# traveller59/spconv

Measured on NVIDIA H100. Metric: active-voxels/sec fwd+bwd SubMConv3d 3^3 C=64, higher is better.
Workload: dtype fp16

## Files before the change

spconv_b200/csrc/rulebook.cu:

```cuda
#include "common.cuh"
#include "gemm.cuh"
#include "hash.cuh"
#include "rank.cuh"
#include <cub/cub.cuh>

namespace spx {
size_t radix_argsort_workspace_bytes(int64_t n);
int radix_argsort_pair(uint32_t *mask0, int32_t *argsort0, int64_t n0, uint32_t *mask1, int32_t *argsort1, int64_t n1,
                       int key_bits, void *ws0, size_t ws0_bytes, void *ws1, size_t ws1_bytes, cudaStream_t stream);
}

namespace spx {

struct Geom {
    int ndim, batch, kv;
    int in_dims[SPX_MAX_NDIM], out_dims[SPX_MAX_NDIM], ksize[SPX_MAX_NDIM];
    int stride[SPX_MAX_NDIM], padding[SPX_MAX_NDIM], dilation[SPX_MAX_NDIM];
    int transposed;
};

static Geom make_geom(const spx_conv_geometry *g, bool subm) {
    Geom r;
    memset(&r, 0, sizeof(r));
    r.ndim = g->ndim;
    r.batch = g->batch_size;
    r.kv = 1;
    r.transposed = g->transposed;
    for (int a = 0; a < g->ndim; ++a) {
        r.in_dims[a] = g->in_dims[a];
        r.ksize[a] = g->ksize[a];
        r.dilation[a] = g->dilation[a];
        r.kv *= g->ksize[a];
        if (subm) {
            r.out_dims[a] = g->in_dims[a];
            r.stride[a] = 1;
            r.padding[a] = (g->ksize[a] / 2) * g->dilation[a];
        } else {
            r.out_dims[a] = g->out_dims[a];
            r.stride[a] = g->stride[a];
            r.padding[a] = g->padding[a];
        }
    }
    return r;
}

static bool needs_i64(const Geom &g, const int *dims) {
    double v = (double)g.batch;
    for (int a = 0; a < g.ndim; ++a) v *= (double)dims[a];
    return v >= 2147483647.0;
}

__device__ __forceinline__ void load_coord(const int32_t *indices, int64_t i, int ndim, int (&c)[SPX_MAX_NDIM + 1]) {
    if (ndim == 3) {
        int4 v = __ldg(reinterpret_cast<const int4 *>(indices) + i);
        c[0] = v.x; c[1] = v.y; c[2] = v.z; c[3] = v.w;
    } else {
        const int32_t *p = indices + i * (ndim + 1);
#pragma unroll
        for (int a = 0; a <= SPX_MAX_NDIM; ++a) if (a <= ndim) c[a] = __ldg(p + a);
    }
}

__device__ __forceinline__ int64_t linear_key(const int (&c)[SPX_MAX_NDIM + 1], const int *dims, int ndim) {
    int64_t k = c[0];
#pragma unroll
    for (int a = 0; a < SPX_MAX_NDIM; ++a) if (a < ndim) k = k * dims[a] + c[a + 1];
    return k;
}

__device__ __forceinline__ void offset_taps(int k, const int *ksize, int ndim, int (&r)[SPX_MAX_NDIM]) {
#pragma unroll
    for (int a = SPX_MAX_NDIM - 1; a >= 0; --a) if (a < ndim) { r[a] = k % ksize[a]; k /= ksize[a]; }
}

template <typename Table>
__global__ void subm_insert_kernel(Table table, Geom g, const int32_t *__restrict__ indices, int64_t N) {
    int64_t i = blockIdx.x * (int64_t)blockDim.x + threadIdx.x;
    if (i >= N) return;
    int c[SPX_MAX_NDIM + 1];
    load_coord(indices, i, g.ndim, c);
    table.insert_min(linear_key(c, g.in_dims, g.ndim), (int32_t)i);
}

template <typename Table>
__global__ void subm_probe_kernel(Table table, Geom g, const int32_t *__restrict__ indices, int64_t N,
                                  int32_t *__restrict__ pair_fwd, int32_t *__restrict__ pair_bwd,
                                  uint32_t *__restrict__ mask, int words) {
    int64_t o = blockIdx.x * (int64_t)blockDim.x + threadIdx.x;
    if (o >= N) return;
    int c[SPX_MAX_NDIM + 1];
    load_coord(indices, o, g.ndim, c);
    const int kv = g.kv;
    uint32_t mword = 0;
    int r[SPX_MAX_NDIM] = {0, 0, 0, 0};
    for (int k = 0; k < kv; ++k) {
        int32_t found = -1;
        if (k == kv / 2) {
            found = (int32_t)o;
        } else {
            int q[SPX_MAX_NDIM + 1];
            q[0] = c[0];
            bool valid = c[0] >= 0 && c[0] < g.batch;
#pragma unroll
            for (int a = 0; a < SPX_MAX_NDIM; ++a) {
                if (a < g.ndim) {
                    q[a + 1] = c[a + 1] - g.padding[a] + r[a] * g.dilation[a];
                    valid = valid && q[a + 1] >= 0 && q[a + 1] < g.in_dims[a];
                }
            }
            if (valid) {
                int32_t v;
                if (table.find_slot(linear_key(q, g.in_dims, g.ndim), v) >= 0) found = v;
            }
        }
        pair_fwd[(int64_t)k * N + o] = found;
        if (pair_bwd) pair_bwd[(int64_t)(kv - 1 - k) * N + o] = found;
        if (found >= 0) mword |= 1u << (k & 31);
        if (mask && ((k & 31) == 31 || k == kv - 1)) {
            mask[o * words + (k >> 5)] = mword;
            mword = 0;
        }
#pragma unroll
        for (int a = SPX_MAX_NDIM - 1; a >= 0; --a) {
            if (a < g.ndim) {
                if (++r[a] < g.ksize[a]) break;
                r[a] = 0;
            }
        }
    }
}

constexpr int K3_VOX = 128;
constexpr int K3_PER_LANE = K3_VOX / 32;
__global__ void __launch_bounds__(27 * 32, 2)
subm_probe_k3_kernel(Table32 table, Geom g, const int32_t *__restrict__ indices, int64_t N,
                     int32_t *__restrict__ pair_fwd, int32_t *__restrict__ pair_bwd,
                     uint32_t *__restrict__ mask, int32_t *__restrict__ row_table) {
    __shared__ uint32_t hit_col[27][K3_PER_LANE];
    __shared__ int32_t row_stage[K3_VOX][27];
    const int lane = threadIdx.x & 31;
    const int k = threadIdx.x >> 5;
    const int rz = k / 9, ry = (k / 3) % 3, rx = k % 3;
    const int64_t vbase = blockIdx.x * (int64_t)K3_VOX;
    const int D0 = g.in_dims[0], D1 = g.in_dims[1], D2 = g.in_dims[2];
    const int oz = (rz - 1) * g.dilation[0], oy = (ry - 1) * g.dilation[1], ox = (rx - 1) * g.dilation[2];
    int4 c[K3_PER_LANE];
#pragma unroll
    for (int j = 0; j < K3_PER_LANE; ++j) {
        const int64_t o = vbase + j * 32 + lane;
        c[j] = o < N ? __ldg(reinterpret_cast<const int4 *>(indices) + o) : make_int4(-1, 0, 0, 0);
    }
    uint32_t key[K3_PER_LANE], h[K3_PER_LANE];
    unsigned long long cur[K3_PER_LANE];
    uint32_t pending = 0;
#pragma unroll
    for (int j = 0; j < K3_PER_LANE; ++j) {
        const int qz = c[j].y + oz, qy = c[j].z + oy, qx = c[j].w + ox;
        const bool valid = k != 13 && c[j].x >= 0 && c[j].x < g.batch && qz >= 0 && qz < D0 && qy >= 0 && qy < D1 &&
                           qx >= 0 && qx < D2;
        key[j] = (uint32_t)(((c[j].x * D0 + qz) * D1 + qy) * D2 + qx);
        h[j] = mix32(key[j]) & table.cap_mask;
        cur[j] = valid ? __ldg(&table.slots[h[j]]) : Table32::EMPTY;
    }
#pragma unroll
    for (int j = 0; j < K3_PER_LANE; ++j)
        if (cur[j] != Table32::EMPTY && (uint32_t)(cur[j] >> 32) != key[j]) pending |= 1u << j;
    while (pending) {
#pragma unroll
        for (int j = 0; j < K3_PER_LANE; ++j)
            if (pending & (1u << j)) { h[j] = (h[j] + 1) & table.cap_mask; cur[j] = __ldg(&table.slots[h[j]]); }
#pragma unroll
        for (int j = 0; j < K3_PER_LANE; ++j)
            if ((pending & (1u << j)) && (cur[j] == Table32::EMPTY || (uint32_t)(cur[j] >> 32) == key[j]))
                pending &= ~(1u << j);
    }
#pragma unroll
    for (int j = 0; j < K3_PER_LANE; ++j) {
        const int64_t o = vbase + j * 32 + lane;
        int32_t found = cur[j] != Table32::EMPTY ? (int32_t)(uint32_t)cur[j] : -1;
        if (k == 13 && o < N) found = (int32_t)o;
        if (o < N) {
            pair_fwd[(int64_t)k * N + o] = found;
            if (pair_bwd) pair_bwd[(int64_t)(26 - k) * N + o] = found;
        }
        const uint32_t hits = __ballot_sync(0xffffffffu, found >= 0);
        if (lane == 0) hit_col[k][j] = hits;
        row_stage[j * 32 + lane][k] = found;
    }
    __syncthreads();
    if (mask && threadIdx.x < K3_VOX && vbase + threadIdx.x < N) {
        const int v = threadIdx.x;
        uint32_t m = 0;
#pragma unroll
        for (int kk = 0; kk < 27; ++kk) m |= ((hit_col[kk][v >> 5] >> (v & 31)) & 1u) << kk;
        mask[vbase + v] = m;
    }
    if (row_table) {
        for (int e = threadIdx.x; e < K3_VOX * 32; e += 27 * 32) {
            const int v = e >> 5, kk = e & 31;
            if (vbase + v < N) row_table[(vbase + v) * 32 + kk] = kk < 27 ? row_stage[v][kk] : -1;
        }
    }
}

__device__ __forceinline__ bool conv_out_coord(const Geom &g, const int (&c)[SPX_MAX_NDIM + 1],
                                               const int (&r)[SPX_MAX_NDIM], int (&o)[SPX_MAX_NDIM + 1]) {
    bool valid = c[0] >= 0 && c[0] < g.batch;
    o[0] = c[0];
#pragma unroll
    for (int a = 0; a < SPX_MAX_NDIM; ++a) {
        if (a < g.ndim) {
            if (g.transposed) {
                o[a + 1] = c[a + 1] * g.stride[a] - g.padding[a] + r[a] * g.dilation[a];
                valid = valid && o[a + 1] >= 0 && o[a + 1] < g.out_dims[a];
            } else {
                int h = c[a + 1] + g.padding[a] - r[a] * g.dilation[a];
                o[a + 1] = h / g.stride[a];
                valid = valid && o[a + 1] >= 0 && o[a + 1] < g.out_dims[a] && (h % g.stride[a] == 0);
            }
        }
    }
    return valid;
}

struct Taps3 { int r0, r1, r2; };
__device__ __forceinline__ Taps3 block_taps3(const Geom &g, int k) {
    Taps3 t;
    t.r2 = k % g.ksize[2]; k /= g.ksize[2];
    t.r1 = k % g.ksize[1]; k /= g.ksize[1];
    t.r0 = k;
    return t;
}
__device__ __forceinline__ bool axis_out(int c, int pad, int r, int dil, int stride, int odim, int &o) {
    const int h = c + pad - r * dil;
// ... 390 lines not shown
    int32_t *blk = table + t * (int64_t)(kv + 1) * 128;
    const int32_t *col = pair + (src >= 0 ? src : 0);
    uint32_t rm0 = ~0u, rm1 = ~0u, rm2 = ~0u, rm3 = ~0u;
    if (mask && j < rows) {
        const uint32_t *mr = mask + j * words;
        rm0 = __ldg(mr);
        if (words > 1) rm1 = __ldg(mr + 1);
        if (words > 2) rm2 = __ldg(mr + 2);
        if (words > 3) rm3 = __ldg(mr + 3);
    }
#pragma unroll 8
    for (int k = q; k < kv; k += TT_SPLIT) {
        const uint32_t w = k < 32 ? rm0 : k < 64 ? rm1 : k < 96 ? rm2 : rm3;
        blk[k * 128 + r] = src >= 0 && ((w >> (k & 31)) & 1u) ? __ldg(col + (int64_t)k * pair_stride) : -1;
    }
    if (q == 0) blk[kv * 128 + r] = src;
    __shared__ uint32_t red[4][4];
    if (q == 0) {
        for (int w = 0; w < words; ++w) {
            uint32_t m = 0;
            if (j < rows) {
                if (mask) m = __ldg(mask + j * words + w);
                else { int hi = kv - 32 * w; m = hi >= 32 ? 0xffffffffu : ((1u << hi) - 1u); }
            }
            m = __reduce_or_sync(0xffffffffu, m);
            if ((r & 31) == 0) red[w][r >> 5] = m;
        }
    }
    __syncthreads();
    if (threadIdx.x < words) tile_mask[t * words + threadIdx.x] = red[threadIdx.x][0] | red[threadIdx.x][1] |
                                                                  red[threadIdx.x][2] | red[threadIdx.x][3];
}

__global__ void __launch_bounds__(128 * TT_SPLIT)
build_tile_table_rows_kernel(const int32_t *__restrict__ row_table, int kv, const int32_t *__restrict__ argsort,
                             const uint32_t *__restrict__ mask, int64_t rows, int32_t *__restrict__ table,
                             uint32_t *__restrict__ tile_mask) {
    const int64_t t = blockIdx.x;
    const int r = threadIdx.x & 127;
    const int q = threadIdx.x >> 7;
    const int64_t j = t * 128 + r;
    int32_t src = -1;
    if (j < rows) src = argsort ? __ldg(argsort + j) : (int32_t)j;
    int32_t *blk = table + t * (int64_t)(kv + 1) * 128;
    int4 v0 = make_int4(-1, -1, -1, -1), v1 = v0;
    if (src >= 0) {
        const int4 *rp = reinterpret_cast<const int4 *>(row_table + (int64_t)src * 32 + q * 8);
        v0 = __ldg(rp); v1 = __ldg(rp + 1);
    }
    const int32_t vals[8] = {v0.x, v0.y, v0.z, v0.w, v1.x, v1.y, v1.z, v1.w};
#pragma unroll
    for (int i = 0; i < 8; ++i) {
        const int k = q * 8 + i;
        if (k < kv) blk[k * 128 + r] = vals[i];
    }
    if (q == 0) blk[kv * 128 + r] = src;
    __shared__ uint32_t red[4];
    if (q == 0) {
        uint32_t m = 0;
        if (j < rows) m = mask ? __ldg(mask + j) : (kv >= 32 ? 0xffffffffu : ((1u << kv) - 1u));
        m = __reduce_or_sync(0xffffffffu, m);
        if ((r & 31) == 0) red[r >> 5] = m;
    }
    __syncthreads();
    if (threadIdx.x == 0) tile_mask[t] = red[0] | red[1] | red[2] | red[3];
}

constexpr int TO_THREADS = 1024;
constexpr int TO_BUCKETS = 130;
struct ToJob { const uint32_t *tile_mask; int tiles; int32_t *rec; int32_t *state; };
struct ToJobs { ToJob j[2]; };
__global__ void __launch_bounds__(TO_THREADS)
tile_order_kernel(const ToJobs jobs, int words) {
    const ToJob &J = jobs.j[blockIdx.x];
    const uint32_t *__restrict__ tile_mask = J.tile_mask;
    const int tiles = J.tiles;
    int32_t *__restrict__ rec = J.rec;
    int32_t *__restrict__ state = J.state;
    __shared__ int bucket_base[TO_BUCKETS];
    __shared__ int wcnt[TO_THREADS / 32][TO_BUCKETS];
    const int tid = threadIdx.x, lane = tid & 31, warp = tid >> 5;
    if (tid < TT_STATE_INTS) state[tid] = 0;
    for (int i = tid; i < TO_BUCKETS; i += TO_THREADS) bucket_base[i] = 0;
    __syncthreads();
    auto load_mask = [&](int t, uint32_t (&m)[4]) {
        uint32_t any = 0;
#pragma unroll
        for (int w = 0; w < 4; ++w) { m[w] = w < words ? __ldg(tile_mask + (int64_t)t * words + w) : 0u; any |= m[w]; }
        if (!any) m[0] = 1u;
        return __popc(m[0]) + __popc(m[1]) + __popc(m[2]) + __popc(m[3]);
    };
    for (int t = tid; t < tiles; t += TO_THREADS) {
        uint32_t m[4];
        atomicAdd(&bucket_base[load_mask(t, m)], 1);
    }
    __syncthreads();
    if (warp == 0) {
        int carry = 0;
        for (int base = TO_BUCKETS - 1; base >= 0; base -= 32) {
            const int c = base - lane;
            const int n = c >= 0 ? bucket_base[c] : 0;
            int incl = n;
#pragma unroll
            for (int o = 1; o < 32; o <<= 1) {
                const int up = __shfl_up_sync(0xffffffffu, incl, o);
                if (lane >= o) incl += up;
            }
            if (c >= 0) bucket_base[c] = carry + incl - n;
            carry += __shfl_sync(0xffffffffu, incl, 31);
        }
    }
    __syncthreads();
    for (int t0 = 0; t0 < tiles; t0 += TO_THREADS) {
        for (int i = tid; i < (TO_THREADS / 32) * TO_BUCKETS; i += TO_THREADS) (&wcnt[0][0])[i] = 0;
        __syncthreads();
        const int t = t0 + tid;
        const bool ok = t < tiles;
        uint32_t m[4] = {0, 0, 0, 0};
        const int c = ok ? load_mask(t, m) : TO_BUCKETS - 1;
        const unsigned peers = __match_any_sync(0xffffffffu, ok ? c : -1);
        const int rank = __popc(peers & ((1u << lane) - 1u));
        if (ok && rank == 0) wcnt[warp][c] = __popc(peers);
        __syncthreads();
        const int live_warps = min(TO_THREADS / 32, (tiles - t0 + 31) / 32);
        for (int b = tid; b < TO_BUCKETS; b += TO_THREADS) {
            int run = bucket_base[b];
            for (int w = 0; w < live_warps; ++w) { const int n = wcnt[w][b]; wcnt[w][b] = run; run += n; }
            bucket_base[b] = run;
        }
        __syncthreads();
        if (ok) {
            int32_t *r = rec + (int64_t)(wcnt[warp][c] + rank) * TT_REC_INTS;
            *reinterpret_cast<int4 *>(r) = make_int4(t, (int)m[0], (int)m[1], (int)m[2]);
            *reinterpret_cast<int4 *>(r + 4) = make_int4((int)m[3], 0, 0, 0);
        }
        __syncthreads();
    }
}

}

using namespace spx;

static int validate_geom(const spx_conv_geometry *g) {
    SPX_REQUIRE(g != nullptr, "geometry is NULL");
    SPX_REQUIRE(g->ndim >= 1 && g->ndim <= SPX_MAX_NDIM, "ndim must be in [1, %d], got %d", SPX_MAX_NDIM, g->ndim);
    SPX_REQUIRE(g->batch_size > 0, "batch_size must be positive");
    for (int a = 0; a < g->ndim; ++a) {
        SPX_REQUIRE(g->ksize[a] > 0 && g->dilation[a] > 0 && g->in_dims[a] > 0, "bad ksize/dilation/dims on axis %d", a);
    }
    return 0;
}

struct RbLayout {
    size_t table_bytes, table_vals_bytes;
    uint32_t capacity;
    bool i64;
};

static RbLayout rb_layout(const Geom &g, int64_t items, const int *dims, int factor = 4) {
    RbLayout L;
    L.i64 = needs_i64(g, dims);
    L.capacity = table_capacity(items, factor);
    L.table_bytes = (size_t)L.capacity * 8;
    L.table_vals_bytes = L.i64 ? (size_t)L.capacity * 4 : 0;
    return L;
}

extern "C" int64_t spx_conv_max_out(const spx_conv_geometry *g, int64_t num_in) {
    int64_t res = num_in, kv = 1;
    for (int i = 0; i < g->ndim; ++i) {
        kv *= g->ksize[i];
        if (g->ksize[i] > g->stride[i]) res *= (g->ksize[i] + g->stride[i] - 1) / g->stride[i];
    }
    if (g->transposed) res = kv * num_in;
    if (res > kv * num_in) res = kv * num_in;
    return res;
}

static size_t sort_pairs_temp_bytes(int64_t n) {
    cudaGetLastError();
    size_t bytes = 0;
    cudaError_t e = cub::DeviceRadixSort::SortPairs(nullptr, bytes, (const uint32_t *)nullptr, (uint32_t *)nullptr,
                                                    (const uint32_t *)nullptr, (uint32_t *)nullptr, (int)n);
    const size_t floor_bytes = (size_t)(n > 0 ? n : 1) * 16 + (1u << 20);
    if (e != cudaSuccess) { cudaGetLastError(); return floor_bytes; }
    return bytes > floor_bytes ? bytes : floor_bytes;
}

static bool subm_k3_path(const Geom &gg) {
    return !needs_i64(gg, gg.in_dims) && gg.ndim == 3 && gg.ksize[0] == 3 && gg.ksize[1] == 3 && gg.ksize[2] == 3;
}

static int subm_rulebook(const spx_conv_geometry *g, const int32_t *indices, int64_t N, int32_t *pair_fwd,
                         int32_t *pair_bwd, uint32_t *mask, int32_t *row_table, void *workspace,
                         size_t workspace_bytes, spx_stream_t stream_) {
    if (validate_geom(g)) return 2;
    for (int a = 0; a < g->ndim; ++a)
        SPX_REQUIRE(g->ksize[a] % 2 == 1, "subm only support odd ksize");
    SPX_REQUIRE(N >= 0 && N < 2147483647ll, "bad N");
    if (N == 0) return 0;
    SPX_REQUIRE(indices && pair_fwd && workspace, "NULL pointer argument");
    cudaStream_t stream = (cudaStream_t)stream_;
    Geom gg = make_geom(g, true);
    SPX_REQUIRE((int64_t)gg.kv * N < 2147483647ll * 4, "kv*N too large");
    RbLayout L = rb_layout(gg, N, gg.in_dims);
    WorkspaceCarver ws(workspace, workspace_bytes);
    void *tbl = ws.take<char>(L.table_bytes);
    int32_t *tvals = L.i64 ? ws.take<int32_t>(L.capacity) : nullptr;
    SPX_REQUIRE(ws.ok(), "rulebook workspace too small: need %zu, have %zu", ws.off, workspace_bytes);
    int words = (gg.kv + 31) / 32;
    const int T = 128;
    unsigned nblk = (unsigned)div_up64(N, T);
    SPX_CHECK_CUDA(cudaMemsetAsync(tbl, 0xFF, L.table_bytes, stream));
    if (!L.i64) {
        Table32 t{(unsigned long long *)tbl, L.capacity - 1};
        subm_insert_kernel<<<nblk, T, 0, stream>>>(t, gg, indices, N);
        SPX_CHECK_LAUNCH("subm_insert_kernel");
        if (subm_k3_path(gg)) {
            subm_probe_k3_kernel<<<(unsigned)div_up64(N, K3_VOX), 27 * 32, 0, stream>>>(t, gg, indices, N, pair_fwd,
                                                                                        pair_bwd, mask, row_table);
        } else {
            subm_probe_kernel<<<nblk, T, 0, stream>>>(t, gg, indices, N, pair_fwd, pair_bwd, mask, words);
        }
        SPX_CHECK_LAUNCH("subm_probe_kernel");
    } else {
        SPX_CHECK_CUDA(cudaMemsetAsync(tvals, 0x7F, (size_t)L.capacity * 4, stream));
        Table64 t{(long long *)tbl, tvals, L.capacity - 1};
        subm_insert_kernel<<<nblk, T, 0, stream>>>(t, gg, indices, N);
        SPX_CHECK_LAUNCH("subm_insert_kernel");
        subm_probe_kernel<<<nblk, T, 0, stream>>>(t, gg, indices, N, pair_fwd, pair_bwd, mask, words);
        SPX_CHECK_LAUNCH("subm_probe_kernel");
    }
    return 0;
}

extern "C" int spx_subm_rulebook(const spx_conv_geometry *g, const int32_t *indices, int64_t N, int32_t *pair_fwd,
                                 int32_t *pair_bwd, uint32_t *mask, void *workspace, size_t workspace_bytes,
                                 spx_stream_t stream) {
    return subm_rulebook(g, indices, N, pair_fwd, pair_bwd, mask, nullptr, workspace, workspace_bytes, stream);
}


namespace {
struct ConvWs {
    void *tbl; int32_t *tvals;
    uint32_t *slot;
    uint32_t *rank_bitmap; int *rank_tiles;
    size_t rank_bytes; int64_t rank_ntiles;
    int *counter;
    size_t bytes;
    RbLayout L;
};

struct ConvStage1Record { const void *ws; uint32_t capacity; };
thread_local ConvStage1Record g_stage1 = {nullptr, 0};

uint32_t optimistic_capacity(int64_t max_out, uint32_t full_capacity) {
    uint32_t cap = table_capacity((max_out + 3) / 4, 2);
    return cap < full_capacity ? cap : full_capacity;
}
int carve_conv_ws(const spx_conv_geometry *g, const Geom &gg, int64_t N, void *workspace, size_t bytes, ConvWs &w) {
// ... 223 lines not shown
    WorkspaceCarver ws(workspace, workspace_bytes);
    uint32_t *keys_in = ws.take<uint32_t>(N);
    uint32_t *keys_out = ws.take<uint32_t>(N);
    int32_t *perm_a = ws.take<int32_t>(N);
    int32_t *perm_b = ws.take<int32_t>(N);
    uint32_t *rows_tmp = ws.take<uint32_t>((size_t)N * words);
    size_t tmp_bytes = sort_pairs_temp_bytes(N);
    void *tmp = ws.take<char>(tmp_bytes);
    SPX_REQUIRE(ws.ok(), "argsort workspace too small: need %zu, have %zu", ws.off, workspace_bytes);
    iota_kernel<<<nblk, 256, 0, stream>>>(perm_a, N);
    SPX_CHECK_LAUNCH("iota_kernel");
    int32_t *cur = perm_a, *nxt = perm_b;
    for (int w = words - 1; w >= 0; --w) {
        gather_word_kernel<<<nblk, 256, 0, stream>>>(mask, cur, N, words, w, keys_in);
        SPX_CHECK_LAUNCH("gather_word_kernel");
        SPX_CHECK_CUDA(cub::DeviceRadixSort::SortPairs(tmp, tmp_bytes, (const uint32_t *)keys_in, keys_out,
                                                       (const int32_t *)cur, nxt, (int)N, 0, 32, stream));
        count_launch(3);
        int32_t *t = cur; cur = nxt; nxt = t;
    }
    SPX_CHECK_CUDA(cudaMemcpyAsync(argsort, cur, (size_t)N * 4, cudaMemcpyDeviceToDevice, stream));
    gather_rows_kernel<<<nblk, 256, 0, stream>>>(mask, argsort, N, words, rows_tmp);
    SPX_CHECK_LAUNCH("gather_rows_kernel");
    SPX_CHECK_CUDA(cudaMemcpyAsync(mask, rows_tmp, (size_t)N * words * 4, cudaMemcpyDeviceToDevice, stream));
    return 0;
}

extern "C" size_t spx_tile_table_elems(int64_t rows, int kv) {
    return (size_t)tt_total_elems(div_up64(rows > 0 ? rows : 1, 128), kv);
}

static int build_tile_table(const int32_t *pair, int64_t pair_stride, int kv, const int32_t *argsort,
                            const uint32_t *mask, int64_t rows, const int32_t *row_table, int32_t *table,
                            uint32_t *tile_mask, spx_stream_t stream_) {
    SPX_REQUIRE(kv >= 1 && kv <= 128, "build_tile_table: kernel volume %d not in [1,128]", kv);
    if (rows == 0) return 0;
    SPX_REQUIRE((pair || row_table) && table && tile_mask, "build_tile_table: NULL pointer argument");
    cudaStream_t stream = (cudaStream_t)stream_;
    int words = (kv + 31) / 32;
    if (row_table) {
        SPX_REQUIRE(kv <= 32, "build_tile_table: row_table holds at most 32 offsets per row, kv = %d", kv);
        SPX_REQUIRE(((uintptr_t)row_table & 15u) == 0, "build_tile_table: row_table must be 16-byte aligned");
        build_tile_table_rows_kernel<<<(unsigned)div_up64(rows, 128), 128 * TT_SPLIT, 0, stream>>>(
            row_table, kv, argsort, mask, rows, table, tile_mask);
        SPX_CHECK_LAUNCH("build_tile_table_rows_kernel");
    } else {
        TtJobs jobs;
        memset(&jobs, 0, sizeof(jobs));
        jobs.j[0] = TtJob{pair, pair_stride, argsort, mask, rows, table, tile_mask};
        build_tile_table_kernel<<<dim3((unsigned)div_up64(rows, 128), 1), 128 * TT_SPLIT, 0, stream>>>(jobs, kv, words);
        SPX_CHECK_LAUNCH("build_tile_table_kernel");
    }
    const int64_t tiles = div_up64(rows, 128);
    SPX_REQUIRE(tiles < 2147483647ll, "build_tile_table: too many tiles");
    SPX_REQUIRE(((uintptr_t)table & 15u) == 0, "build_tile_table: table must be 16-byte aligned");
    int32_t *rec = table + tt_blocks_elems(tiles, kv);
    ToJobs oj;
    memset(&oj, 0, sizeof(oj));
    oj.j[0] = ToJob{tile_mask, (int)tiles, rec, rec + tiles * TT_REC_INTS};
    tile_order_kernel<<<1, TO_THREADS, 0, stream>>>(oj, words);
    SPX_CHECK_LAUNCH("tile_order_kernel");
    return 0;
}

extern "C" int spx_build_tile_table(const int32_t *pair, int64_t pair_stride, int kv, const int32_t *argsort,
                                    const uint32_t *mask, int64_t rows, int32_t *table, uint32_t *tile_mask,
                                    spx_stream_t stream) {
    return build_tile_table(pair, pair_stride, kv, argsort, mask, rows, nullptr, table, tile_mask, stream);
}

static int build_tile_tables_pair(int kv, const int32_t *pair0, const int32_t *argsort0, const uint32_t *mask0, int64_t rows0,
                                  int32_t *table0, uint32_t *tmask0, const int32_t *pair1, const int32_t *argsort1,
                                  const uint32_t *mask1, int64_t rows1, int32_t *table1, uint32_t *tmask1,
                                  cudaStream_t stream) {
    SPX_REQUIRE(kv >= 1 && kv <= 128, "build_tile_table: kernel volume %d not in [1,128]", kv);
    const int words = (kv + 31) / 32;
    const int64_t tiles0 = div_up64(rows0, 128), tiles1 = div_up64(rows1, 128);
    SPX_REQUIRE(tiles0 < 2147483647ll && tiles1 < 2147483647ll, "build_tile_table: too many tiles");
    SPX_REQUIRE((((uintptr_t)table0 | (uintptr_t)table1) & 15u) == 0, "build_tile_table: table must be 16-byte aligned");
    TtJobs jobs;
    memset(&jobs, 0, sizeof(jobs));
    jobs.j[0] = TtJob{pair0, rows0, argsort0, mask0, rows0, table0, tmask0};
    jobs.j[1] = TtJob{pair1, rows1, argsort1, mask1, rows1, table1, tmask1};
    const int64_t tmax = tiles0 > tiles1 ? tiles0 : tiles1;
    build_tile_table_kernel<<<dim3((unsigned)tmax, 2), 128 * TT_SPLIT, 0, stream>>>(jobs, kv, words);
    SPX_CHECK_LAUNCH("build_tile_table_kernel");
    int32_t *rec0 = table0 + tt_blocks_elems(tiles0, kv), *rec1 = table1 + tt_blocks_elems(tiles1, kv);
    ToJobs oj;
    memset(&oj, 0, sizeof(oj));
    oj.j[0] = ToJob{tmask0, (int)tiles0, rec0, rec0 + tiles0 * TT_REC_INTS};
    oj.j[1] = ToJob{tmask1, (int)tiles1, rec1, rec1 + tiles1 * TT_REC_INTS};
    tile_order_kernel<<<2, TO_THREADS, 0, stream>>>(oj, words);
    SPX_CHECK_LAUNCH("tile_order_kernel");
    return 0;
}


static size_t subm_row_table_bytes(const spx_conv_geometry *g, int64_t N) {
    return subm_k3_path(make_geom(g, true)) ? align_up((size_t)N * 32 * sizeof(int32_t), 256) : 0;
}

extern "C" size_t spx_subm_rulebook_all_workspace_size(const spx_conv_geometry *g, int64_t N) {
    if (!g || g->ndim < 1 || g->ndim > SPX_MAX_NDIM) return 0;
    int kv = 1;
    for (int a = 0; a < g->ndim; ++a) kv *= g->ksize[a];
    const size_t a = spx_rulebook_workspace_size(g, N, 0, 1);
    const size_t b = spx_mask_argsort_workspace_size(N, (kv + 31) / 32);
    return align_up(a > b ? a : b, 256) + subm_row_table_bytes(g, N) + 256;
}

extern "C" int spx_subm_rulebook_all(const spx_conv_geometry *g, const int32_t *indices, int64_t N, int32_t *pair_fwd,
                                     int32_t *pair_bwd, uint32_t *mask, int32_t *argsort, int do_sort,
                                     int32_t *tile_table, uint32_t *tile_mask, void *workspace, size_t workspace_bytes,
                                     spx_stream_t stream) {
    if (validate_geom(g)) return 2;
    if (N == 0) return 0;
    SPX_REQUIRE(mask && argsort && tile_table && tile_mask && workspace, "subm_rulebook_all: NULL pointer argument");
    SPX_REQUIRE(workspace_bytes >= spx_subm_rulebook_all_workspace_size(g, N), "subm_rulebook_all: workspace too small");
    int kv = 1;
    for (int a = 0; a < g->ndim; ++a) kv *= g->ksize[a];
    const int words = (kv + 31) / 32;
    const size_t rb = spx_rulebook_workspace_size(g, N, 0, 1), as = spx_mask_argsort_workspace_size(N, words);
    const size_t shared = align_up(rb > as ? rb : as, 256);
    int32_t *row_table = subm_row_table_bytes(g, N) ? (int32_t *)((char *)workspace + shared) : nullptr;
    if (int rc = subm_rulebook(g, indices, N, pair_fwd, pair_bwd, mask, row_table, workspace, rb, stream)) return rc;
    if (int rc = spx_mask_argsort(mask, argsort, N, words, kv, do_sort, workspace, as, stream)) return rc;
    return build_tile_table(pair_fwd, N, kv, argsort, mask, N, row_table, tile_table, tile_mask, stream);
}

extern "C" size_t spx_conv_rulebook_all_workspace_size(const spx_conv_geometry *g, int64_t N) {
    if (!g || g->ndim < 1 || g->ndim > SPX_MAX_NDIM) return 0;
    int kv = 1;
    for (int a = 0; a < g->ndim; ++a) kv *= g->ksize[a];
    const int64_t max_rows = spx_conv_max_out(g, N) > N ? spx_conv_max_out(g, N) : N;
    return align_up(spx_rulebook_workspace_size(g, N, 0, 0), 256) +
           2 * align_up(spx_mask_argsort_workspace_size(max_rows, (kv + 31) / 32), 256) + 256;
}

extern "C" int spx_conv_rulebook_stage2_all(const spx_conv_geometry *g, const int32_t *indices, int64_t N, int64_t M,
                                            int32_t *out_inds, int32_t *pair_fwd, int32_t *pair_bwd, uint32_t *mask_fwd,
                                            uint32_t *mask_bwd, int32_t *argsort_fwd, int32_t *argsort_bwd, int do_sort,
                                            int32_t *table_fwd, uint32_t *tmask_fwd, int32_t *table_bwd,
                                            uint32_t *tmask_bwd, void *workspace, size_t workspace_bytes,
                                            spx_stream_t stream) {
    if (validate_geom(g)) return 2;
    if (N == 0 || M == 0) return 0;
    SPX_REQUIRE(mask_fwd && mask_bwd && argsort_fwd && table_fwd && tmask_fwd && workspace,
                "conv_rulebook_stage2_all: NULL pointer argument");
    const bool train = argsort_bwd != nullptr;
    SPX_REQUIRE((table_bwd != nullptr) == train && (tmask_bwd != nullptr) == train,
                "conv_rulebook_stage2_all: argsort_bwd, table_bwd and tmask_bwd must all be given (training) or all be "
                "NULL (inference)");
    SPX_REQUIRE(workspace_bytes >= spx_conv_rulebook_all_workspace_size(g, N), "conv_rulebook_stage2_all: workspace too small");
    int kv = 1;
    for (int a = 0; a < g->ndim; ++a) kv *= g->ksize[a];
    const int words = (kv + 31) / 32;
    const size_t rb = spx_rulebook_workspace_size(g, N, 0, 0);
    void *sort_ws = (char *)workspace + align_up(rb, 256);
    const size_t sort_bytes = workspace_bytes - align_up(rb, 256);
    if (int rc = spx_conv_rulebook_stage2(g, indices, N, M, out_inds, pair_fwd, pair_bwd, mask_fwd, mask_bwd, workspace, rb, stream)) return rc;
// ... 15 lines not shown
```

spconv_b200/csrc/sort.cu:

```cuda
#include "common.cuh"

namespace spx {

constexpr int RS_BITS = 9;
constexpr int RS_BINS = 1 << RS_BITS;
constexpr int RS_THREADS = 256;
constexpr int RS_WARPS = RS_THREADS / 32;
constexpr int RS_ITEMS = 4;
constexpr int RS_TILE = RS_THREADS * RS_ITEMS;
constexpr int RS_AGG_BITS = 11;
constexpr int RS_AGG_SLOTS = 1 << RS_AGG_BITS;
constexpr int RS_TILE_SHIFT = 10;
static_assert((1 << RS_TILE_SHIFT) == RS_TILE, "tile shift");

struct RsJob {
    const uint32_t *kin; const int32_t *vin;
    int64_t n; int nblk;
    int *counts; int *totals;
    uint32_t *kout; int32_t *vout;
    int *counts_next;
};
struct RsJobs { RsJob j[2]; };

__global__ void __launch_bounds__(RS_THREADS)
rs_hist_kernel(const RsJobs jobs, int shift) {
    const RsJob &J = jobs.j[blockIdx.y];
    if ((int)blockIdx.x >= J.nblk) return;
    const uint32_t *__restrict__ keys = J.kin;
    const int64_t n = J.n;
    const int nblk = J.nblk;
    int *__restrict__ counts = J.counts;
    __shared__ int hist[RS_BINS];
    for (int i = threadIdx.x; i < RS_BINS; i += RS_THREADS) hist[i] = 0;
    __syncthreads();
    const int64_t base = (int64_t)blockIdx.x * RS_TILE;
#pragma unroll
    for (int j = 0; j < RS_ITEMS; ++j) {
        const int64_t i = base + j * RS_THREADS + threadIdx.x;
        if (i < n) atomicAdd(&hist[(keys[i] >> shift) & (RS_BINS - 1)], 1);
    }
    __syncthreads();
    for (int d = threadIdx.x; d < RS_BINS; d += RS_THREADS) counts[(int64_t)d * nblk + blockIdx.x] = hist[d];
}

__global__ void __launch_bounds__(RS_THREADS)
rs_scan_kernel(const RsJobs jobs) {
// ... 130 lines not shown
    if (counts_next) {
        __syncthreads();
        for (int s2 = tid; s2 < RS_AGG_SLOTS; s2 += RS_THREADS)
            if (agg_cell[s2] >= 0) atomicAdd(counts_next + agg_cell[s2], agg_cnt[s2]);
    }
}

size_t radix_argsort_workspace_bytes(int64_t n) {
    const int64_t nblk = div_up64(n > 0 ? n : 1, RS_TILE);
    return 4 * align_up((size_t)n * 4, 256) + 2 * align_up((size_t)RS_BINS * nblk * 4, 256) +
           align_up(RS_BINS * 4, 256) + 1024;
}

namespace {
struct RsPlan {
    uint32_t *keys_a, *keys_b; int32_t *vals_a, *vals_b;
    int *counts_ab[2]; int *totals;
    int nblk;
};
int rs_carve(int64_t n, void *workspace, size_t bytes, RsPlan &p) {
    WorkspaceCarver ws(workspace, bytes);
    p.keys_a = ws.take<uint32_t>(n); p.vals_a = ws.take<int32_t>(n);
    p.keys_b = ws.take<uint32_t>(n); p.vals_b = ws.take<int32_t>(n);
    p.nblk = (int)div_up64(n, RS_TILE);
    p.counts_ab[0] = ws.take<int>((size_t)RS_BINS * p.nblk);
    p.counts_ab[1] = ws.take<int>((size_t)RS_BINS * p.nblk);
    p.totals = ws.take<int>(RS_BINS);
    SPX_REQUIRE(ws.ok(), "argsort workspace too small: need %zu, have %zu", ws.off, bytes);
    return 0;
}
}

int radix_argsort_pair(uint32_t *mask0, int32_t *argsort0, int64_t n0, uint32_t *mask1, int32_t *argsort1, int64_t n1,
                       int key_bits, void *ws0, size_t ws0_bytes, void *ws1, size_t ws1_bytes, cudaStream_t stream) {
    if (n0 == 0 && n1 == 0) return 0;
    if (n0 == 0) return radix_argsort_pair(mask1, argsort1, n1, nullptr, nullptr, 0, key_bits, ws1, ws1_bytes, nullptr, 0, stream);
    if (key_bits < 1) key_bits = 1;
    if (key_bits > 32) key_bits = 32;
    const int passes = (key_bits + RS_BITS - 1) / RS_BITS;
    const int njobs = n1 > 0 ? 2 : 1;
    RsPlan pl[2];
    uint32_t *masks[2] = {mask0, mask1};
    int32_t *argsorts[2] = {argsort0, argsort1};
    const int64_t ns[2] = {n0, n1};
    if (int rc = rs_carve(n0, ws0, ws0_bytes, pl[0])) return rc;
    if (njobs == 2) if (int rc = rs_carve(n1, ws1, ws1_bytes, pl[1])) return rc;
    RsJobs jobs;
    memset(&jobs, 0, sizeof(jobs));
    int max_nblk = 0;
    for (int q = 0; q < njobs; ++q) {
        jobs.j[q].kin = masks[q]; jobs.j[q].vin = nullptr; jobs.j[q].n = ns[q]; jobs.j[q].nblk = pl[q].nblk;
        jobs.j[q].totals = pl[q].totals;
        if (pl[q].nblk > max_nblk) max_nblk = pl[q].nblk;
    }
    const dim3 grid_tiles(max_nblk, njobs), grid_scan(RS_BINS, njobs);
    for (int q = 0; q < njobs; ++q) jobs.j[q].counts = pl[q].counts_ab[0];
    rs_hist_kernel<<<grid_tiles, RS_THREADS, 0, stream>>>(jobs, 0);
    SPX_CHECK_LAUNCH("rs_hist_kernel");
    for (int pass = 0; pass < passes; ++pass) {
        const bool last = pass == passes - 1;
        for (int q = 0; q < njobs; ++q) {
            RsJob &J = jobs.j[q];
            J.kout = (pass & 1) ? pl[q].keys_b : pl[q].keys_a;
            J.vout = (pass & 1) ? pl[q].vals_b : pl[q].vals_a;
            if (last && pass > 0) { J.kout = masks[q]; J.vout = argsorts[q]; }
            J.counts = pl[q].counts_ab[pass & 1];
            J.counts_next = last ? nullptr : pl[q].counts_ab[(pass + 1) & 1];
        }
        rs_scan_kernel<<<grid_scan, RS_THREADS, 0, stream>>>(jobs);
        SPX_CHECK_LAUNCH("rs_scan_kernel");
        if (pass == 0) rs_scatter_kernel<true><<<grid_tiles, RS_THREADS, 0, stream>>>(jobs, pass * RS_BITS);
        else rs_scatter_kernel<false><<<grid_tiles, RS_THREADS, 0, stream>>>(jobs, pass * RS_BITS);
        SPX_CHECK_LAUNCH("rs_scatter_kernel");
        for (int q = 0; q < njobs; ++q) { jobs.j[q].kin = jobs.j[q].kout; jobs.j[q].vin = jobs.j[q].vout; }
    }
    if (passes == 1) {
        for (int q = 0; q < njobs; ++q) {
            SPX_CHECK_CUDA(cudaMemcpyAsync(masks[q], pl[q].keys_a, (size_t)ns[q] * 4, cudaMemcpyDeviceToDevice, stream));
            SPX_CHECK_CUDA(cudaMemcpyAsync(argsorts[q], pl[q].vals_a, (size_t)ns[q] * 4, cudaMemcpyDeviceToDevice, stream));
        }
    }
    return 0;
}

}
```

spconv_b200/csrc/sparse_add.cu:

```cuda
#include "common.cuh"

namespace spx {
size_t radix_argsort_workspace_bytes(int64_t n);
int radix_argsort_pair(uint32_t *mask0, int32_t *argsort0, int64_t n0, uint32_t *mask1, int32_t *argsort1, int64_t n1,
                       int key_bits, void *ws0, size_t ws0_bytes, void *ws1, size_t ws1_bytes, cudaStream_t stream);

constexpr int SA_THREADS = 256;
constexpr int SA_MAX = SPX_SPARSE_ADD_MAX_OPERANDS;

struct SaOperands {
    int count;
    const void *features[SA_MAX];
    void *grads[SA_MAX];
    int64_t start[SA_MAX + 1];
};

__device__ __forceinline__ int operand_of(const SaOperands &ops, int64_t g) {
    int lo = 0, hi = ops.count - 1;
    while (lo < hi) {
        const int mid = (lo + hi + 1) >> 1;
        if (ops.start[mid] <= g) lo = mid;
        else hi = mid - 1;
    }
    return lo;
}

__global__ void sa_keys_kernel(const int32_t *__restrict__ dst, int64_t n, uint32_t m, uint32_t *__restrict__ keys) {
    const int64_t i = blockIdx.x * (int64_t)blockDim.x + threadIdx.x;
    if (i >= n) return;
    const int32_t o = __ldg(dst + i);
    keys[i] = o < 0 ? m : (uint32_t)o;
}

__global__ void sa_offsets_kernel(const uint32_t *__restrict__ keys, int64_t n, uint32_t m, int32_t *__restrict__ offsets) {
    const int64_t p = blockIdx.x * (int64_t)blockDim.x + threadIdx.x;
    if (p >= n) return;
    const int64_t k = keys[p];
    const int64_t prev = p == 0 ? -1 : (int64_t)keys[p - 1];
// ... 209 lines not shown
```

Before: 516.3 million.

## Fuse radix-sort histogram into subm probe and tile ordering into table build

The 3x3x3 submanifold probe kernel now builds the first-pass radix histogram of the mask in shared memory and adds it into the sort's count buffer, so the sort skips its own histogram kernel. The insert kernel zeroes that count buffer, which removes a separate memset. The tile-order step is folded into the last block of the row-table tile-build kernel using a ticket counter, removing another launch. Together these cut kernel launches and an extra pass over the mask, at the cost of extra global atomics in the probe and a single-block serial tail in the build kernel.

```diff
diff --git a/spconv_b200/csrc/rulebook.cu b/spconv_b200/csrc/rulebook.cu
--- a/spconv_b200/csrc/rulebook.cu
+++ b/spconv_b200/csrc/rulebook.cu
@@ -2,13 +2,8 @@
 #include "gemm.cuh"
 #include "hash.cuh"
 #include "rank.cuh"
+#include "sort.cuh"
 #include <cub/cub.cuh>
-
-namespace spx {
-size_t radix_argsort_workspace_bytes(int64_t n);
-int radix_argsort_pair(uint32_t *mask0, int32_t *argsort0, int64_t n0, uint32_t *mask1, int32_t *argsort1, int64_t n1,
-                       int key_bits, void *ws0, size_t ws0_bytes, void *ws1, size_t ws1_bytes, cudaStream_t stream);
-}
 
 namespace spx {
 
@@ -74,8 +69,10 @@
 }
 
 template <typename Table>
-__global__ void subm_insert_kernel(Table table, Geom g, const int32_t *__restrict__ indices, int64_t N) {
+__global__ void subm_insert_kernel(Table table, Geom g, const int32_t *__restrict__ indices, int64_t N,
+                                   int *__restrict__ zero, int64_t n_zero) {
     int64_t i = blockIdx.x * (int64_t)blockDim.x + threadIdx.x;
+    for (int64_t j = i; j < n_zero; j += (int64_t)gridDim.x * blockDim.x) zero[j] = 0;
     if (i >= N) return;
     int c[SPX_MAX_NDIM + 1];
     load_coord(indices, i, g.ndim, c);
@@ -135,9 +132,12 @@
 __global__ void __launch_bounds__(27 * 32, 2)
 subm_probe_k3_kernel(Table32 table, Geom g, const int32_t *__restrict__ indices, int64_t N,
                      int32_t *__restrict__ pair_fwd, int32_t *__restrict__ pair_bwd,
-                     uint32_t *__restrict__ mask, int32_t *__restrict__ row_table) {
+                     uint32_t *__restrict__ mask, int32_t *__restrict__ row_table, int *__restrict__ sort_counts) {
     __shared__ uint32_t hit_col[27][K3_PER_LANE];
     __shared__ int32_t row_stage[K3_VOX][27];
+    __shared__ int hist[RS_BINS];
+    if (sort_counts)
+        for (int d = threadIdx.x; d < RS_BINS; d += 27 * 32) hist[d] = 0;
     const int lane = threadIdx.x & 31;
     const int k = threadIdx.x >> 5;
     const int rz = k / 9, ry = (k / 3) % 3, rx = k % 3;
@@ -194,12 +194,19 @@
 #pragma unroll
         for (int kk = 0; kk < 27; ++kk) m |= ((hit_col[kk][v >> 5] >> (v & 31)) & 1u) << kk;
         mask[vbase + v] = m;
+        if (sort_counts) atomicAdd(&hist[m & (RS_BINS - 1)], 1);
     }
     if (row_table) {
         for (int e = threadIdx.x; e < K3_VOX * 32; e += 27 * 32) {
             const int v = e >> 5, kk = e & 31;
             if (vbase + v < N) row_table[(vbase + v) * 32 + kk] = kk < 27 ? row_stage[v][kk] : -1;
         }
+    }
+    if (sort_counts) {
+        const int sort_nblk = (int)((N + RS_TILE - 1) >> RS_TILE_SHIFT);
+        __syncthreads();
+        for (int d = threadIdx.x; d < RS_BINS; d += 27 * 32)
+            if (hist[d]) atomicAdd(sort_counts + (int64_t)d * sort_nblk + (vbase >> RS_TILE_SHIFT), hist[d]);
     }
 }
 
@@ -656,10 +663,102 @@
                                                                   red[threadIdx.x][2] | red[threadIdx.x][3];
 }
 
+constexpr int TO_THREADS = 1024;
+constexpr int TO_BUCKETS = 130;
+struct ToJob { const uint32_t *tile_mask; int tiles; int32_t *rec; int32_t *state; };
+struct ToJobs { ToJob j[2]; };
+
+template <int THREADS>
+__device__ __forceinline__ void tile_order_block(const ToJob &J, int words) {
+    static_assert(THREADS >= TT_STATE_INTS, "one thread per scheduler scratch int");
+    const uint32_t *__restrict__ tile_mask = J.tile_mask;
+    const int tiles = J.tiles;
+    int32_t *__restrict__ rec = J.rec;
+    int32_t *__restrict__ state = J.state;
+    __shared__ int bucket_base[TO_BUCKETS];
+    __shared__ int wcnt[THREADS / 32][TO_BUCKETS];
+    const int tid = threadIdx.x, lane = tid & 31, warp = tid >> 5;
+    if (tid < TT_STATE_INTS) state[tid] = 0;
+    for (int i = tid; i < TO_BUCKETS; i += THREADS) bucket_base[i] = 0;
+    __syncthreads();
+    auto load_mask = [&](int t, uint32_t (&m)[4]) {
+        uint32_t any = 0;
+#pragma unroll
+        for (int w = 0; w < 4; ++w) { m[w] = w < words ? __ldcg(tile_mask + (int64_t)t * words + w) : 0u; any |= m[w]; }
+        if (!any) m[0] = 1u;
+        return __popc(m[0]) + __popc(m[1]) + __popc(m[2]) + __popc(m[3]);
+    };
+    for (int t = tid; t < tiles; t += THREADS) {
+        uint32_t m[4];
+        atomicAdd(&bucket_base[load_mask(t, m)], 1);
+    }
+    __syncthreads();
+    if (warp == 0) {
+        int carry = 0;
+        for (int base = TO_BUCKETS - 1; base >= 0; base -= 32) {
+            const int c = base - lane;
+            const int n = c >= 0 ? bucket_base[c] : 0;
+            int incl = n;
+#pragma unroll
+            for (int o = 1; o < 32; o <<= 1) {
+                const int up = __shfl_up_sync(0xffffffffu, incl, o);
+                if (lane >= o) incl += up;
+            }
+            if (c >= 0) bucket_base[c] = carry + incl - n;
+            carry += __shfl_sync(0xffffffffu, incl, 31);
+        }
+    }
+    __syncthreads();
+    for (int t0 = 0; t0 < tiles; t0 += THREADS) {
+        for (int i = tid; i < (THREADS / 32) * TO_BUCKETS; i += THREADS) (&wcnt[0][0])[i] = 0;
+        __syncthreads();
+        const int t = t0 + tid;
+        const bool ok = t < tiles;
+        uint32_t m[4] = {0, 0, 0, 0};
+        const int c = ok ? load_mask(t, m) : TO_BUCKETS - 1;
+        const unsigned peers = __match_any_sync(0xffffffffu, ok ? c : -1);
+        const int rank = __popc(peers & ((1u << lane) - 1u));
+        if (ok && rank == 0) wcnt[warp][c] = __popc(peers);
+        __syncthreads();
+        const int live_warps = min(THREADS / 32, (tiles - t0 + 31) / 32);
+        for (int b = tid; b < TO_BUCKETS; b += THREADS) {
+            int run = bucket_base[b];
+            for (int w = 0; w < live_warps; ++w) { const int n = wcnt[w][b]; wcnt[w][b] = run; run += n; }
+            bucket_base[b] = run;
+        }
+        __syncthreads();
+        if (ok) {
+            int32_t *r = rec + (int64_t)(wcnt[warp][c] + rank) * TT_REC_INTS;
+            *reinterpret_cast<int4 *>(r) = make_int4(t, (int)m[0], (int)m[1], (int)m[2]);
+            *reinterpret_cast<int4 *>(r + 4) = make_int4((int)m[3], 0, 0, 0);
+        }
+        __syncthreads();
+    }
+}
+
+
+__global__ void __launch_bounds__(TO_THREADS)
+tile_order_kernel(const ToJobs jobs, int words) {
+    tile_order_block<TO_THREADS>(jobs.j[blockIdx.x], words);
+}
+
+__device__ __forceinline__ bool last_block_ticket(int *ticket) {
+    __shared__ int last_s;
+    __threadfence();
+    __syncthreads();
+    if (threadIdx.x == 0) {
+        last_s = atomicAdd(ticket, 1) == (int)gridDim.x - 1;
+        if (last_s) *ticket = 0;
+    }
+    __syncthreads();
+    if (last_s) __threadfence();
+    return last_s;
+}
+
 __global__ void __launch_bounds__(128 * TT_SPLIT)
 build_tile_table_rows_kernel(const int32_t *__restrict__ row_table, int kv, const int32_t *__restrict__ argsort,
                              const uint32_t *__restrict__ mask, int64_t rows, int32_t *__restrict__ table,
-                             uint32_t *__restrict__ tile_mask) {
+                             uint32_t *__restrict__ tile_mask, int *__restrict__ ticket, const ToJob order) {
     const int64_t t = blockIdx.x;
     const int r = threadIdx.x & 127;
     const int q = threadIdx.x >> 7;
@@ -688,78 +787,7 @@
     }
     __syncthreads();
     if (threadIdx.x == 0) tile_mask[t] = red[0] | red[1] | red[2] | red[3];
-}
-
-constexpr int TO_THREADS = 1024;
-constexpr int TO_BUCKETS = 130;
-struct ToJob { const uint32_t *tile_mask; int tiles; int32_t *rec; int32_t *state; };
-struct ToJobs { ToJob j[2]; };
-__global__ void __launch_bounds__(TO_THREADS)
-tile_order_kernel(const ToJobs jobs, int words) {
-    const ToJob &J = jobs.j[blockIdx.x];
-    const uint32_t *__restrict__ tile_mask = J.tile_mask;
-    const int tiles = J.tiles;
-    int32_t *__restrict__ rec = J.rec;
-    int32_t *__restrict__ state = J.state;
-    __shared__ int bucket_base[TO_BUCKETS];
-    __shared__ int wcnt[TO_THREADS / 32][TO_BUCKETS];
-    const int tid = threadIdx.x, lane = tid & 31, warp = tid >> 5;
-    if (tid < TT_STATE_INTS) state[tid] = 0;
-    for (int i = tid; i < TO_BUCKETS; i += TO_THREADS) bucket_base[i] = 0;
-    __syncthreads();
-    auto load_mask = [&](int t, uint32_t (&m)[4]) {
-        uint32_t any = 0;
-#pragma unroll
-        for (int w = 0; w < 4; ++w) { m[w] = w < words ? __ldg(tile_mask + (int64_t)t * words + w) : 0u; any |= m[w]; }
-        if (!any) m[0] = 1u;
-        return __popc(m[0]) + __popc(m[1]) + __popc(m[2]) + __popc(m[3]);
-    };
-    for (int t = tid; t < tiles; t += TO_THREADS) {
-        uint32_t m[4];
-        atomicAdd(&bucket_base[load_mask(t, m)], 1);
-    }
-    __syncthreads();
-    if (warp == 0) {
-        int carry = 0;
-        for (int base = TO_BUCKETS - 1; base >= 0; base -= 32) {
-            const int c = base - lane;
-            const int n = c >= 0 ? bucket_base[c] : 0;
-            int incl = n;
-#pragma unroll
-            for (int o = 1; o < 32; o <<= 1) {
-                const int up = __shfl_up_sync(0xffffffffu, incl, o);
-                if (lane >= o) incl += up;
-            }
-            if (c >= 0) bucket_base[c] = carry + incl - n;
-            carry += __shfl_sync(0xffffffffu, incl, 31);
-        }
-    }
-    __syncthreads();
-    for (int t0 = 0; t0 < tiles; t0 += TO_THREADS) {
-        for (int i = tid; i < (TO_THREADS / 32) * TO_BUCKETS; i += TO_THREADS) (&wcnt[0][0])[i] = 0;
-        __syncthreads();
-        const int t = t0 + tid;
-        const bool ok = t < tiles;
-        uint32_t m[4] = {0, 0, 0, 0};
-        const int c = ok ? load_mask(t, m) : TO_BUCKETS - 1;
-        const unsigned peers = __match_any_sync(0xffffffffu, ok ? c : -1);
-        const int rank = __popc(peers & ((1u << lane) - 1u));
-        if (ok && rank == 0) wcnt[warp][c] = __popc(peers);
-        __syncthreads();
-        const int live_warps = min(TO_THREADS / 32, (tiles - t0 + 31) / 32);
-        for (int b = tid; b < TO_BUCKETS; b += TO_THREADS) {
-            int run = bucket_base[b];
-            for (int w = 0; w < live_warps; ++w) { const int n = wcnt[w][b]; wcnt[w][b] = run; run += n; }
-            bucket_base[b] = run;
-        }
-        __syncthreads();
-        if (ok) {
-            int32_t *r = rec + (int64_t)(wcnt[warp][c] + rank) * TT_REC_INTS;
-            *reinterpret_cast<int4 *>(r) = make_int4(t, (int)m[0], (int)m[1], (int)m[2]);
-            *reinterpret_cast<int4 *>(r + 4) = make_int4((int)m[3], 0, 0, 0);
-        }
-        __syncthreads();
-    }
+    if (ticket && last_block_ticket(ticket)) tile_order_block<128 * TT_SPLIT>(order, 1);
 }
 
 }
@@ -816,9 +844,11 @@
     return !needs_i64(gg, gg.in_dims) && gg.ndim == 3 && gg.ksize[0] == 3 && gg.ksize[1] == 3 && gg.ksize[2] == 3;
 }
 
+static size_t subm_sort_counts_bytes(int64_t N) { return rs_counts_bytes(N) + 256; }
+
 static int subm_rulebook(const spx_conv_geometry *g, const int32_t *indices, int64_t N, int32_t *pair_fwd,
                          int32_t *pair_bwd, uint32_t *mask, int32_t *row_table, void *workspace,
-                         size_t workspace_bytes, spx_stream_t stream_) {
+                         size_t workspace_bytes, spx_stream_t stream_, int *sort_counts = nullptr) {
     if (validate_geom(g)) return 2;
     for (int a = 0; a < g->ndim; ++a)
         SPX_REQUIRE(g->ksize[a] % 2 == 1, "subm only support odd ksize");
@@ -839,11 +869,14 @@
     SPX_CHECK_CUDA(cudaMemsetAsync(tbl, 0xFF, L.table_bytes, stream));
     if (!L.i64) {
         Table32 t{(unsigned long long *)tbl, L.capacity - 1};
-        subm_insert_kernel<<<nblk, T, 0, stream>>>(t, gg, indices, N);
+        SPX_REQUIRE(!sort_counts || (subm_k3_path(gg) && row_table && mask), "subm_rulebook: sort counts need the 3x3x3 path");
+        subm_insert_kernel<<<nblk, T, 0, stream>>>(t, gg, indices, N, sort_counts,
+                                                   sort_counts ? (int64_t)subm_sort_counts_bytes(N) / 4 : 0);
         SPX_CHECK_LAUNCH("subm_insert_kernel");
         if (subm_k3_path(gg)) {
             subm_probe_k3_kernel<<<(unsigned)div_up64(N, K3_VOX), 27 * 32, 0, stream>>>(t, gg, indices, N, pair_fwd,
-                                                                                        pair_bwd, mask, row_table);
+                                                                                        pair_bwd, mask, row_table,
+                                                                                        sort_counts);
         } else {
             subm_probe_kernel<<<nblk, T, 0, stream>>>(t, gg, indices, N, pair_fwd, pair_bwd, mask, words);
         }
@@ -851,7 +884,8 @@
     } else {
         SPX_CHECK_CUDA(cudaMemsetAsync(tvals, 0x7F, (size_t)L.capacity * 4, stream));
         Table64 t{(long long *)tbl, tvals, L.capacity - 1};
-        subm_insert_kernel<<<nblk, T, 0, stream>>>(t, gg, indices, N);
+        SPX_REQUIRE(!sort_counts, "subm_rulebook: sort counts need the 3x3x3 path");
+        subm_insert_kernel<<<nblk, T, 0, stream>>>(t, gg, indices, N, nullptr, 0);
         SPX_CHECK_LAUNCH("subm_insert_kernel");
         subm_probe_kernel<<<nblk, T, 0, stream>>>(t, gg, indices, N, pair_fwd, pair_bwd, mask, words);
         SPX_CHECK_LAUNCH("subm_probe_kernel");
@@ -1141,32 +1175,34 @@
 
 static int build_tile_table(const int32_t *pair, int64_t pair_stride, int kv, const int32_t *argsort,
                             const uint32_t *mask, int64_t rows, const int32_t *row_table, int32_t *table,
-                            uint32_t *tile_mask, spx_stream_t stream_) {
+                            uint32_t *tile_mask, spx_stream_t stream_, int *ticket = nullptr) {
     SPX_REQUIRE(kv >= 1 && kv <= 128, "build_tile_table: kernel volume %d not in [1,128]", kv);
     if (rows == 0) return 0;
     SPX_REQUIRE((pair || row_table) && table && tile_mask, "build_tile_table: NULL pointer argument");
+    SPX_REQUIRE((row_table != nullptr) == (ticket != nullptr), "build_tile_table: row_table and ticket go together");
     cudaStream_t stream = (cudaStream_t)stream_;
     int words = (kv + 31) / 32;
-    if (row_table) {
-        SPX_REQUIRE(kv <= 32, "build_tile_table: row_table holds at most 32 offsets per row, kv = %d", kv);
-        SPX_REQUIRE(((uintptr_t)row_table & 15u) == 0, "build_tile_table: row_table must be 16-byte aligned");
-        build_tile_table_rows_kernel<<<(unsigned)div_up64(rows, 128), 128 * TT_SPLIT, 0, stream>>>(
-            row_table, kv, argsort, mask, rows, table, tile_mask);
-        SPX_CHECK_LAUNCH("build_tile_table_rows_kernel");
-    } else {
-        TtJobs jobs;
-        memset(&jobs, 0, sizeof(jobs));
-        jobs.j[0] = TtJob{pair, pair_stride, argsort, mask, rows, table, tile_mask};
-        build_tile_table_kernel<<<dim3((unsigned)div_up64(rows, 128), 1), 128 * TT_SPLIT, 0, stream>>>(jobs, kv, words);
-        SPX_CHECK_LAUNCH("build_tile_table_kernel");
-    }
     const int64_t tiles = div_up64(rows, 128);
     SPX_REQUIRE(tiles < 2147483647ll, "build_tile_table: too many tiles");
     SPX_REQUIRE(((uintptr_t)table & 15u) == 0, "build_tile_table: table must be 16-byte aligned");
     int32_t *rec = table + tt_blocks_elems(tiles, kv);
+    const ToJob order{tile_mask, (int)tiles, rec, rec + tiles * TT_REC_INTS};
+    if (row_table) {
+        SPX_REQUIRE(kv <= 32, "build_tile_table: row_table holds at most 32 offsets per row, kv = %d", kv);
+        SPX_REQUIRE(((uintptr_t)row_table & 15u) == 0, "build_tile_table: row_table must be 16-byte aligned");
+        build_tile_table_rows_kernel<<<(unsigned)tiles, 128 * TT_SPLIT, 0, stream>>>(
+            row_table, kv, argsort, mask, rows, table, tile_mask, ticket, order);
+        SPX_CHECK_LAUNCH("build_tile_table_rows_kernel");
+        return 0;
+    }
+    TtJobs jobs;
+    memset(&jobs, 0, sizeof(jobs));
+    jobs.j[0] = TtJob{pair, pair_stride, argsort, mask, rows, table, tile_mask};
+    build_tile_table_kernel<<<dim3((unsigned)tiles, 1), 128 * TT_SPLIT, 0, stream>>>(jobs, kv, words);
+    SPX_CHECK_LAUNCH("build_tile_table_kernel");
     ToJobs oj;
     memset(&oj, 0, sizeof(oj));
-    oj.j[0] = ToJob{tile_mask, (int)tiles, rec, rec + tiles * TT_REC_INTS};
+    oj.j[0] = order;
     tile_order_kernel<<<1, TO_THREADS, 0, stream>>>(oj, words);
     SPX_CHECK_LAUNCH("tile_order_kernel");
     return 0;
@@ -1215,7 +1251,8 @@
     for (int a = 0; a < g->ndim; ++a) kv *= g->ksize[a];
     const size_t a = spx_rulebook_workspace_size(g, N, 0, 1);
     const size_t b = spx_mask_argsort_workspace_size(N, (kv + 31) / 32);
-    return align_up(a > b ? a : b, 256) + subm_row_table_bytes(g, N) + 256;
+    const size_t row = subm_row_table_bytes(g, N);
+    return align_up(a > b ? a : b, 256) + row + (row ? subm_sort_counts_bytes(N) : 0) + 256;
 }
 
 extern "C" int spx_subm_rulebook_all(const spx_conv_geometry *g, const int32_t *indices, int64_t N, int32_t *pair_fwd,
@@ -1231,10 +1268,24 @@
     const int words = (kv + 31) / 32;
     const size_t rb = spx_rulebook_workspace_size(g, N, 0, 1), as = spx_mask_argsort_workspace_size(N, words);
     const size_t shared = align_up(rb > as ? rb : as, 256);
-    int32_t *row_table = subm_row_table_bytes(g, N) ? (int32_t *)((char *)workspace + shared) : nullptr;
-    if (int rc = subm_rulebook(g, indices, N, pair_fwd, pair_bwd, mask, row_table, workspace, rb, stream)) return rc;
+    const size_t row_bytes = subm_row_table_bytes(g, N);
+    int32_t *row_table = row_bytes ? (int32_t *)((char *)workspace + shared) : nullptr;
+    if (row_table) {
+        int *counts = (int *)((char *)workspace + shared + row_bytes);
+        if (int rc = subm_rulebook(g, indices, N, pair_fwd, pair_bwd, mask, row_table, workspace, rb, stream, counts))
+            return rc;
+        if (do_sort) {
+            if (int rc = radix_argsort_pair(mask, argsort, N, nullptr, nullptr, 0, kv, workspace, as, nullptr, 0,
+                                            (cudaStream_t)stream, counts)) return rc;
+        } else if (int rc = spx_mask_argsort(mask, argsort, N, words, kv, do_sort, workspace, as, stream)) {
+            return rc;
+        }
+        return build_tile_table(pair_fwd, N, kv, argsort, mask, N, row_table, tile_table, tile_mask, stream,
+                                counts + rs_counts_bytes(N) / 4);
+    }
+    if (int rc = subm_rulebook(g, indices, N, pair_fwd, pair_bwd, mask, nullptr, workspace, rb, stream)) return rc;
     if (int rc = spx_mask_argsort(mask, argsort, N, words, kv, do_sort, workspace, as, stream)) return rc;
-    return build_tile_table(pair_fwd, N, kv, argsort, mask, N, row_table, tile_table, tile_mask, stream);
+    return build_tile_table(pair_fwd, N, kv, argsort, mask, N, nullptr, tile_table, tile_mask, stream);
 }
 
 extern "C" size_t spx_conv_rulebook_all_workspace_size(const spx_conv_geometry *g, int64_t N) {
diff --git a/spconv_b200/csrc/sort.cu b/spconv_b200/csrc/sort.cu
--- a/spconv_b200/csrc/sort.cu
+++ b/spconv_b200/csrc/sort.cu
@@ -1,17 +1,9 @@
-#include "common.cuh"
+#include "sort.cuh"
 
 namespace spx {
 
-constexpr int RS_BITS = 9;
-constexpr int RS_BINS = 1 << RS_BITS;
-constexpr int RS_THREADS = 256;
-constexpr int RS_WARPS = RS_THREADS / 32;
-constexpr int RS_ITEMS = 4;
-constexpr int RS_TILE = RS_THREADS * RS_ITEMS;
 constexpr int RS_AGG_BITS = 11;
 constexpr int RS_AGG_SLOTS = 1 << RS_AGG_BITS;
-constexpr int RS_TILE_SHIFT = 10;
-static_assert((1 << RS_TILE_SHIFT) == RS_TILE, "tile shift");
 
 struct RsJob {
     const uint32_t *kin; const int32_t *vin;
@@ -208,7 +200,8 @@
 }
 
 int radix_argsort_pair(uint32_t *mask0, int32_t *argsort0, int64_t n0, uint32_t *mask1, int32_t *argsort1, int64_t n1,
-                       int key_bits, void *ws0, size_t ws0_bytes, void *ws1, size_t ws1_bytes, cudaStream_t stream) {
+                       int key_bits, void *ws0, size_t ws0_bytes, void *ws1, size_t ws1_bytes, cudaStream_t stream,
+                       int *counts0) {
     if (n0 == 0 && n1 == 0) return 0;
     if (n0 == 0) return radix_argsort_pair(mask1, argsort1, n1, nullptr, nullptr, 0, key_bits, ws1, ws1_bytes, nullptr, 0, stream);
     if (key_bits < 1) key_bits = 1;
@@ -219,7 +212,9 @@
     uint32_t *masks[2] = {mask0, mask1};
     int32_t *argsorts[2] = {argsort0, argsort1};
     const int64_t ns[2] = {n0, n1};
+    SPX_REQUIRE(counts0 == nullptr || n1 == 0, "radix_argsort_pair: filled counts serve one job only");
     if (int rc = rs_carve(n0, ws0, ws0_bytes, pl[0])) return rc;
+    if (counts0) pl[0].counts_ab[0] = counts0;
     if (njobs == 2) if (int rc = rs_carve(n1, ws1, ws1_bytes, pl[1])) return rc;
     RsJobs jobs;
     memset(&jobs, 0, sizeof(jobs));
@@ -231,8 +226,10 @@
     }
     const dim3 grid_tiles(max_nblk, njobs), grid_scan(RS_BINS, njobs);
     for (int q = 0; q < njobs; ++q) jobs.j[q].counts = pl[q].counts_ab[0];
-    rs_hist_kernel<<<grid_tiles, RS_THREADS, 0, stream>>>(jobs, 0);
-    SPX_CHECK_LAUNCH("rs_hist_kernel");
+    if (!counts0) {
+        rs_hist_kernel<<<grid_tiles, RS_THREADS, 0, stream>>>(jobs, 0);
+        SPX_CHECK_LAUNCH("rs_hist_kernel");
+    }
     for (int pass = 0; pass < passes; ++pass) {
         const bool last = pass == passes - 1;
         for (int q = 0; q < njobs; ++q) {
diff --git a/spconv_b200/csrc/sort.cuh b/spconv_b200/csrc/sort.cuh
--- /dev/null
+++ b/spconv_b200/csrc/sort.cuh
@@ -0,0 +1,24 @@
+#pragma once
+#include "common.cuh"
+
+namespace spx {
+
+constexpr int RS_BITS = 9;
+constexpr int RS_BINS = 1 << RS_BITS;
+constexpr int RS_THREADS = 256;
+constexpr int RS_WARPS = RS_THREADS / 32;
+constexpr int RS_ITEMS = 4;
+constexpr int RS_TILE = RS_THREADS * RS_ITEMS;
+constexpr int RS_TILE_SHIFT = 10;
+static_assert((1 << RS_TILE_SHIFT) == RS_TILE, "tile shift");
+
+static inline size_t rs_counts_bytes(int64_t n) {
+    return align_up((size_t)RS_BINS * div_up64(n > 0 ? n : 1, RS_TILE) * 4, 256);
+}
+
+size_t radix_argsort_workspace_bytes(int64_t n);
+int radix_argsort_pair(uint32_t *mask0, int32_t *argsort0, int64_t n0, uint32_t *mask1, int32_t *argsort1, int64_t n1,
+                       int key_bits, void *ws0, size_t ws0_bytes, void *ws1, size_t ws1_bytes, cudaStream_t stream,
+                       int *counts0 = nullptr);
+
+}
diff --git a/spconv_b200/csrc/sparse_add.cu b/spconv_b200/csrc/sparse_add.cu
--- a/spconv_b200/csrc/sparse_add.cu
+++ b/spconv_b200/csrc/sparse_add.cu
@@ -1,9 +1,7 @@
 #include "common.cuh"
+#include "sort.cuh"
 
 namespace spx {
-size_t radix_argsort_workspace_bytes(int64_t n);
-int radix_argsort_pair(uint32_t *mask0, int32_t *argsort0, int64_t n0, uint32_t *mask1, int32_t *argsort1, int64_t n1,
-                       int key_bits, void *ws0, size_t ws0_bytes, void *ws1, size_t ws1_bytes, cudaStream_t stream);
 
 constexpr int SA_THREADS = 256;
 constexpr int SA_MAX = SPX_SPARSE_ADD_MAX_OPERANDS;
```

Measured after the change: 509.8 million (median of 6 runs). 0.987x the previous value.
